# yeyupiaoling/MASR

Measured on NVIDIA H100. Metric: audio_seconds_per_second, higher is better.
Workload: dtype f32 (GEMMs: fp16x2-split operands on wgmma, fp32 accumulate; fp32-grade results)

## Files before the change

### masr_b200/csrc/ffn_tc.cu

```cuda
#include <cuda.h>
#include <cuda_fp16.h>
#include <stdlib.h>
#include <string.h>

#include "tc_common.cuh"

namespace masr {

namespace {

constexpr int FM = 64;
constexpr int FD = 256;
constexpr int FHC = 128;
constexpr int FBK = 32;
constexpr int F_STAGES = 3;
constexpr int F_STAGE_BYTES = 32768;
constexpr int F_H_BYTES = FM * FHC * 2 * 2;
constexpr int F_SUM_BYTES = FM * FD * 4;
constexpr int F_THREADS = 384;
constexpr int F_PRODUCER_REGS = 40, F_CONSUMER_REGS = 232;
constexpr uint32_t F_TX_A = 2 * FM * FBK * 2 + 2 * FHC * FBK * 2;
constexpr uint32_t F_TX_B = 2 * FD * FBK * 2;
constexpr size_t kFfnSmem = F_STAGES * F_STAGE_BYTES + 2 * F_H_BYTES + F_SUM_BYTES + 1024 + 256;
static_assert(kFfnSmem <= 232448, "ffn_tc shared memory exceeds the 227 KB per-CTA limit of sm_90");
static_assert(F_PRODUCER_REGS * 128 + F_CONSUMER_REGS * 256 <= 65536, "register file of the SM");

struct FfnMaps {
    CUtensorMap xh, xl;
    CUtensorMap w1h, w1l;
    CUtensorMap w2h, w2l;
};

struct FfnParams {
    const void* w[4];
    const float* b1;
    const float* b2;
    float* x;
    int64_t ldx;
    int M, F;
    float alpha;
    int flags;
};

constexpr int FFN_NO_LOADS = 1, FFN_NO_MMA = 2, FFN_NO_EPILOGUE = 4;

__device__ __forceinline__ void wgmma_m64n64k16_ss(float (&d)[32], uint64_t da, uint64_t db, uint32_t scale_d) {
    asm volatile(
        "{\n\t"
        ".reg .pred p;\n\t"
        "setp.ne.b32 p, %34, 0;\n\t"
        "wgmma.mma_async.sync.aligned.m64n64k16.f32.f16.f16 "
        "{%0, %1, %2, %3, %4, %5, %6, %7, %8, %9, %10, %11, %12, %13, %14, %15, "
        "%16, %17, %18, %19, %20, %21, %22, %23, %24, %25, %26, %27, %28, %29, %30, %31}, %32, %33, p, 1, 1, 0, 0;\n\t"
        "}"
        : "+f"(d[0]), "+f"(d[1]), "+f"(d[2]), "+f"(d[3]), "+f"(d[4]), "+f"(d[5]), "+f"(d[6]), "+f"(d[7]), "+f"(d[8]),
          "+f"(d[9]), "+f"(d[10]), "+f"(d[11]), "+f"(d[12]), "+f"(d[13]), "+f"(d[14]), "+f"(d[15]), "+f"(d[16]),
          "+f"(d[17]), "+f"(d[18]), "+f"(d[19]), "+f"(d[20]), "+f"(d[21]), "+f"(d[22]), "+f"(d[23]), "+f"(d[24]),
          "+f"(d[25]), "+f"(d[26]), "+f"(d[27]), "+f"(d[28]), "+f"(d[29]), "+f"(d[30]), "+f"(d[31])
        : "l"(da), "l"(db), "r"(scale_d));
}

__device__ __forceinline__ void bar_consumers() { asm volatile("bar.sync 1, 256;" ::: "memory"); }

template <bool PROBE>
__global__ void __launch_bounds__(F_THREADS, 1) ffn_tc_kernel(const __grid_constant__ FfnMaps maps, FfnParams p) {
    const bool no_loads = PROBE && (p.flags & FFN_NO_LOADS), no_mma = PROBE && (p.flags & FFN_NO_MMA);
    const bool no_epilogue = PROBE && (p.flags & FFN_NO_EPILOGUE);
    extern __shared__ uint8_t smem_raw[];
    uint8_t* smem = reinterpret_cast<uint8_t*>((reinterpret_cast<uintptr_t>(smem_raw) + 1023) & ~uintptr_t(1023));
    uint8_t* hbuf = smem + F_STAGES * F_STAGE_BYTES;
    uint8_t* sum = hbuf + 2 * F_H_BYTES;
    uint64_t* full_bar = reinterpret_cast<uint64_t*>(sum + F_SUM_BYTES);
    uint64_t* empty_bar = full_bar + F_STAGES;

    const int warp = threadIdx.x >> 5, lane = threadIdx.x & 31;
    const int nrb = (p.M + FM - 1) / FM;
    const int nch = p.F / FHC;

    if (warp == 8 && lane == 0) {
        tma_prefetch_desc(&maps.xh); tma_prefetch_desc(&maps.xl); tma_prefetch_desc(&maps.w1h);
        tma_prefetch_desc(&maps.w1l); tma_prefetch_desc(&maps.w2h); tma_prefetch_desc(&maps.w2l);
        for (int s = 0; s < F_STAGES; ++s) { mbar_init(&full_bar[s], 1); mbar_init(&empty_bar[s], 8); }
        asm volatile("fence.mbarrier_init.release.cluster;" ::: "memory");
        const uint32_t wbytes = (uint32_t)p.F * FD * 2;
        const uint32_t share = ((wbytes + gridDim.x - 1) / gridDim.x + 15) & ~15u;
        const uint32_t off = share * blockIdx.x;
        if (!no_loads && off < wbytes)
            for (int t = 0; t < 4; ++t)
                asm volatile("cp.async.bulk.prefetch.L2.global [%0], %1;"
                             ::"l"(static_cast<const uint8_t*>(p.w[t]) + off), "r"(min(share, wbytes - off)) : "memory");
    }
    __syncthreads();
    pdl_wait();
    pdl_launch_dependents();

    if (warp >= 8) {
        setmaxnreg_dec<F_PRODUCER_REGS>();
        if (warp == 8 && elect_one_sync()) {
            uint32_t kg = 0;
            auto acquire = [&](uint32_t tx) {
                const uint32_t s = kg % F_STAGES;
                mbar_wait(&empty_bar[s], ((kg / F_STAGES) & 1) ^ 1);
                if (no_loads) mbar_arrive(&full_bar[s]);
                else mbar_expect_tx(&full_bar[s], tx);
                ++kg;
                return s;
            };
            auto load_a = [&](int m0, int j) {
                const int n0 = j * FHC;
#pragma unroll 1
                for (int kb = 0; kb < FD / FBK; ++kb) {
                    const uint32_t s = acquire(F_TX_A);
                    if (no_loads) continue;
                    uint8_t* st = smem + s * F_STAGE_BYTES;
                    tma_load_2d(&maps.xh, &full_bar[s], st, kb * FBK, m0);
                    tma_load_2d(&maps.xl, &full_bar[s], st + 4096, kb * FBK, m0);
                    tma_load_2d(&maps.w1h, &full_bar[s], st + 8192, kb * FBK, n0);
                    tma_load_2d(&maps.w1l, &full_bar[s], st + 16384, kb * FBK, n0);
                }
            };
            for (int rb = blockIdx.x; rb < nrb; rb += gridDim.x) {
                load_a(rb * FM, 0);
                for (int j = 0; j < nch; ++j) {
                    if (j + 1 < nch) load_a(rb * FM, j + 1);
#pragma unroll 1
                    for (int kb = 0; kb < FHC / FBK; ++kb) {
                        const uint32_t s = acquire(F_TX_B);
                        if (no_loads) continue;
                        uint8_t* st = smem + s * F_STAGE_BYTES;
                        tma_load_2d(&maps.w2h, &full_bar[s], st, j * FHC + kb * FBK, 0);
                        tma_load_2d(&maps.w2l, &full_bar[s], st + F_STAGE_BYTES / 2, j * FHC + kb * FBK, 0);
                    }
                }
            }
        }
        __syncwarp();
    } else {
        setmaxnreg_inc<F_CONSUMER_REGS>();
        const int wg = warp >> 2, wi = warp & 3, q = lane & 3;
        const int tid = threadIdx.x & 127;
        const uint32_t h_base = smem_u32(hbuf);
        const uint32_t sum_base = smem_u32(sum) + wg * (F_SUM_BYTES / 2) + tid * 8;
        const uint32_t is_lane0 = lane == 0;
        auto release = [&](uint32_t s) {
            asm volatile("{\n\t.reg .pred p;\n\tsetp.ne.u32 p, %1, 0;\n\t@p mbarrier.arrive.shared::cta.b64 _, [%0];\n\t}"
                         ::"r"(smem_u32(&empty_bar[s])), "r"(is_lane0) : "memory");
        };
        float acc1[32], cor1[32], acc2[64], cor2[64];
        uint32_t kg = 0;
        int pend = -1;
        auto next_stage = [&]() {
            const uint32_t s = kg % F_STAGES;
            mbar_wait(&full_bar[s], (kg / F_STAGES) & 1);
            ++kg;
            return s;
        };
        auto retire = [&](uint32_t s) {
            wgmma_wait<1>();
            reg_fence(acc1); reg_fence(cor1); reg_fence(acc2); reg_fence(cor2);
            if (pend >= 0) release((uint32_t)pend);
            pend = (int)s;
        };
        auto phase_a = [&](int kb_begin, int kb_end) {
#pragma unroll 1
            for (int kb = kb_begin; kb < kb_end; ++kb) {
                const uint32_t s = next_stage();
                const uint32_t sa = smem_u32(smem + s * F_STAGE_BYTES);
                const uint64_t dXh = gmma_desc_sw64(sa), dXl = gmma_desc_sw64(sa + 4096);
                const uint64_t dWh = gmma_desc_sw64(sa + 8192 + wg * 4096), dWl = gmma_desc_sw64(sa + 16384 + wg * 4096);
                reg_fence(acc1); reg_fence(cor1);
                wgmma_fence();
#pragma unroll
                for (int ks = 0; ks < FBK / 16; ++ks) {
                    if (no_mma) break;
                    const uint64_t adv = (uint64_t)(ks * 2);
                    const uint32_t first = (kb | ks) ? 1u : 0u;
                    wgmma_m64n64k16_ss(acc1, dXh + adv, dWh + adv, first);
                    wgmma_m64n64k16_ss(cor1, dXh + adv, dWl + adv, first);
                    wgmma_m64n64k16_ss(cor1, dXl + adv, dWh + adv, 1u);
                }
                wgmma_commit();
                retire(s);
            }
        };
        auto phase_b = [&](int j, uint32_t hb, int kb) {
            const uint32_t s = next_stage();
            const uint32_t sa = smem_u32(smem + s * F_STAGE_BYTES);
            const uint64_t dWh = gmma_desc_sw64(sa + wg * 8192), dWl = gmma_desc_sw64(sa + F_STAGE_BYTES / 2 + wg * 8192);
            const uint64_t dHh = gmma_desc_sw64(hb + kb * 8192), dHl = gmma_desc_sw64(hb + kb * 8192 + 4096);
            reg_fence(acc2); reg_fence(cor2);
            wgmma_fence();
#pragma unroll
            for (int ks = 0; ks < FBK / 16; ++ks) {
                if (no_mma) break;
                const uint64_t adv = (uint64_t)(ks * 2);
                wgmma_m64n128k16_ss(acc2, dHh + adv, dWh + adv, ((j & 1) | kb | ks) ? 1u : 0u);
                wgmma_m64n128k16_ss(cor2, dHh + adv, dWl + adv, (j | kb | ks) ? 1u : 0u);
                wgmma_m64n128k16_ss(cor2, dHl + adv, dWh + adv, 1u);
            }
            wgmma_commit();
            retire(s);
        };
        const int r_lo = 16 * wi + (lane >> 2);
        auto load_b1 = [&](int j, int sl, float2 (&bb)[2]) {
            const float* b = p.b1 + j * FHC + 64 * wg + 16 * sl + 2 * q;
            bb[0] = __ldg(reinterpret_cast<const float2*>(b));
            bb[1] = __ldg(reinterpret_cast<const float2*>(b + 8));
        };
        auto store_hidden = [&](uint32_t hb, int sl, const float2 (&bb)[2]) {
            if (no_epilogue) return;
#pragma unroll
            for (int i = 2 * sl; i < 2 * sl + 2; ++i)
#pragma unroll
                for (int hh = 0; hh < 2; ++hh) {
                    float v0 = fmaf(cor1[4 * i + 2 * hh], kLoInv, acc1[4 * i + 2 * hh]);
                    float v1 = fmaf(cor1[4 * i + 2 * hh + 1], kLoInv, acc1[4 * i + 2 * hh + 1]);
                    v0 += bb[i - 2 * sl].x; v1 += bb[i - 2 * sl].y;
                    float e0, e1;
                    mul2(e0, e1, v0, v1, -1.4426950408889634f, -1.4426950408889634f);
                    e0 = ex2_approx(e0); e1 = ex2_approx(e1);
                    add2(e0, e1, e0, e1, 1.0f, 1.0f);
                    e0 = rcp_approx(e0); e1 = rcp_approx(e1);
                    mul2(v0, v1, v0, v1, e0, e1);
                    __half2 h2, l2;
                    split_f16x2(v0, v1, h2, l2);
                    const int r = r_lo + 8 * hh, c = 64 * wg + 8 * i + 2 * q;
                    const uint32_t a = hb + (c >> 5) * 8192 + r * 64 + ((((c & 31) >> 3) ^ ((r >> 1) & 3)) << 4) + (c & 7) * 2;
                    asm volatile("st.shared.b32 [%0], %1;" ::"r"(a), "r"(*reinterpret_cast<uint32_t*>(&h2)) : "memory");
                    asm volatile("st.shared.b32 [%0], %1;" ::"r"(a + 4096), "r"(*reinterpret_cast<uint32_t*>(&l2)) : "memory");
                }
        };
        auto fence_h = [&]() { asm volatile("fence.proxy.async.shared::cta;" ::: "memory"); };
        auto drain = [&]() {
            wgmma_wait<0>();
            reg_fence(acc1); reg_fence(cor1); reg_fence(acc2); reg_fence(cor2);
            if (pend >= 0) release((uint32_t)pend);
            pend = -1;
        };

        auto add_sum = [&](int j) {
#pragma unroll
            for (int i = 0; i < 16; ++i)
#pragma unroll
                for (int hh = 0; hh < 2; ++hh) {
                    float x0 = acc2[4 * i + 2 * hh], x1 = acc2[4 * i + 2 * hh + 1];
                    const uint32_t a = sum_base + (i * 2 + hh) * 1024;
                    if (j > 1) {
                        float s0, s1;
                        asm volatile("ld.shared.v2.f32 {%0, %1}, [%2];" : "=f"(s0), "=f"(s1) : "r"(a) : "memory");
                        x0 = s0 + x0; x1 = s1 + x1;
                    }
                    asm volatile("st.shared.v2.f32 [%0], {%1, %2};" ::"r"(a), "f"(x0), "f"(x1) : "memory");
                }
        };
        auto write_out = [&](int m0) {
            const float* b2 = p.b2 + 128 * wg + 2 * q;
#pragma unroll
            for (int i = 0; i < 16; ++i) {
                const float2 bv = __ldg(reinterpret_cast<const float2*>(b2 + 8 * i));
#pragma unroll
                for (int hh = 0; hh < 2; ++hh) {
                    float x0 = acc2[4 * i + 2 * hh], x1 = acc2[4 * i + 2 * hh + 1];
                    if (nch > 2) {
                        float s0, s1;
                        asm volatile("ld.shared.v2.f32 {%0, %1}, [%2];" : "=f"(s0), "=f"(s1) : "r"(sum_base + (i * 2 + hh) * 1024) : "memory");
                        x0 = s0 + x0; x1 = s1 + x1;
                    }
                    x0 = fmaf(cor2[4 * i + 2 * hh], kLoInv, x0);
                    x1 = fmaf(cor2[4 * i + 2 * hh + 1], kLoInv, x1);
                    x0 += bv.x; x1 += bv.y;
                    const int row = m0 + r_lo + 8 * hh;
                    if (row < p.M) {
                        float2* xp = reinterpret_cast<float2*>(p.x + (int64_t)row * p.ldx + 128 * wg + 8 * i + 2 * q);
                        const float2 r = *xp;
                        x0 = r.x + p.alpha * x0;
                        x1 = r.y + p.alpha * x1;
                        *xp = make_float2(x0, x1);
                    }
                }
            }
        };

#pragma unroll 1
        for (int rb = blockIdx.x; rb < nrb; rb += gridDim.x) {
            phase_a(0, FD / FBK);
            drain();
#pragma unroll
            for (int sl = 0; sl < 4; ++sl) {
                float2 bb[2];
                load_b1(0, sl, bb);
                store_hidden(h_base, sl, bb);
            }
            fence_h();
            phase_a(0, FD / FBK);
            drain();
            bar_consumers();
#pragma unroll 1
            for (int j = 0; j < nch; ++j) {
                const bool next = j + 1 < nch, a2 = j + 2 < nch;
                const uint32_t hb = h_base + (j & 1) * F_H_BYTES, hn = h_base + ((j + 1) & 1) * F_H_BYTES;
#pragma unroll
                for (int kb = 0; kb < FHC / FBK; ++kb) {
                    float2 bb[2];
                    if (next) load_b1(j + 1, kb, bb);
                    phase_b(j, hb, kb);
                    if (next) store_hidden(hn, kb, bb);
                }
                if (next) fence_h();
                if (a2) phase_a(0, 1);
                else drain();
                if ((j & 1) && j + 1 < nch) add_sum(j);
                if (j == nch - 1) write_out(rb * FM);
                if (a2) phase_a(1, FD / FBK);
                if (next) bar_consumers();
                drain();
            }
        }
    }
    __syncthreads();
}

int ffn_map(CUtensorMap* map, const void* ptr, int64_t rows, int64_t K, int64_t ld, int box_rows) {
    EncodeTiledFn fn = get_encode_fn();
    if (!fn) { set_last_error("cuTensorMapEncodeTiled entry point unavailable"); return MASR_ERR_INTERNAL; }
    cuuint64_t dims[2] = {(cuuint64_t)K, (cuuint64_t)rows};
    cuuint64_t strides[1] = {(cuuint64_t)ld * 2};
    cuuint32_t box[2] = {(cuuint32_t)FBK, (cuuint32_t)box_rows};
    cuuint32_t estr[2] = {1, 1};
    CUresult r = fn(map, CU_TENSOR_MAP_DATA_TYPE_FLOAT16, 2, const_cast<void*>(ptr), dims, strides, box, estr,
                    CU_TENSOR_MAP_INTERLEAVE_NONE, CU_TENSOR_MAP_SWIZZLE_64B, CU_TENSOR_MAP_L2_PROMOTION_L2_128B,
                    CU_TENSOR_MAP_FLOAT_OOB_FILL_NONE);
    if (r != CUDA_SUCCESS) { set_last_error("cuTensorMapEncodeTiled failed (%d) rows=%lld K=%lld ld=%lld", (int)r, (long long)rows, (long long)K, (long long)ld); return MASR_ERR_INTERNAL; }
    return MASR_OK;
}

bool g_ffn_attr_set[64] = {false};

}

}

using namespace masr;

extern "C" int masr_ffn_tc_f16x2(const void* Ah, const void* Al, int64_t lda, const void* W1h, const void* W1l, const float* b1,
                                 const void* W2h, const void* W2l, const float* b2, float* x, int64_t ldx, int M, int D, int F,
                                 float alpha, void* stream) {
    if (M == 0) return MASR_OK;
    MASR_REQUIRE(Ah && Al && W1h && W1l && b1 && W2h && W2l && b2 && x, "masr_ffn_tc_f16x2: null pointer");
    MASR_REQUIRE(M > 0, "masr_ffn_tc_f16x2: M=%d", M);
    MASR_REQUIRE(D == FD, "masr_ffn_tc_f16x2: D=%d unsupported (this build: %d)", D, FD);
    MASR_REQUIRE(F > 0 && F % 256 == 0, "masr_ffn_tc_f16x2: F=%d must be a positive multiple of 256", F);
    MASR_REQUIRE(lda >= D && lda % 8 == 0, "masr_ffn_tc_f16x2: lda=%lld must be >= %d and a multiple of 8", (long long)lda, D);
    MASR_REQUIRE(ldx >= D && ldx % 2 == 0, "masr_ffn_tc_f16x2: ldx=%lld must be >= %d and even", (long long)ldx, D);
    MASR_REQUIRE(((reinterpret_cast<uintptr_t>(Ah) | reinterpret_cast<uintptr_t>(Al) | reinterpret_cast<uintptr_t>(W1h) |
                   reinterpret_cast<uintptr_t>(W1l) | reinterpret_cast<uintptr_t>(W2h) | reinterpret_cast<uintptr_t>(W2l)) & 15) == 0 &&
                 ((reinterpret_cast<uintptr_t>(x) | reinterpret_cast<uintptr_t>(b1) | reinterpret_cast<uintptr_t>(b2)) & 7) == 0,
                 "masr_ffn_tc_f16x2: misaligned pointer");
    FfnMaps maps;
    memset(&maps, 0, sizeof(maps));
    int rc;
    if ((rc = ffn_map(&maps.xh, Ah, M, D, lda, FM))) return rc;
    if ((rc = ffn_map(&maps.xl, Al, M, D, lda, FM))) return rc;
    if ((rc = ffn_map(&maps.w1h, W1h, F, D, D, FHC))) return rc;
    if ((rc = ffn_map(&maps.w1l, W1l, F, D, D, FHC))) return rc;
    if ((rc = ffn_map(&maps.w2h, W2h, D, F, F, FD))) return rc;
    if ((rc = ffn_map(&maps.w2l, W2l, D, F, F, FD))) return rc;
    int dev = 0;
    cudaGetDevice(&dev);
    if (dev < 0 || dev >= 64) dev = 0;
    void (*const kernels[2])(FfnMaps, FfnParams) = {ffn_tc_kernel<false>, ffn_tc_kernel<true>};
    if (!g_ffn_attr_set[dev]) {
        for (auto k : kernels) {
            cudaError_t e = cudaFuncSetAttribute(k, cudaFuncAttributeMaxDynamicSharedMemorySize, (int)kFfnSmem);
            if (e != cudaSuccess) { set_last_error("ffn_tc smem attr: %s", cudaGetErrorString(e)); return (int)e; }
        }
        g_ffn_attr_set[dev] = true;
    }
    int sms = 0;
    if (cudaDeviceGetAttribute(&sms, cudaDevAttrMultiProcessorCount, dev) != cudaSuccess || sms <= 0) sms = 132;
    const int nrb = (M + FM - 1) / FM;
    const char* env = getenv("MASR_FFN_FLAGS");
    const int flags = env ? atoi(env) : 0;
    FfnParams p{{W1h, W1l, W2h, W2l}, b1, b2, x, ldx, M, F, alpha, flags};
    const dim3 grid(nrb < sms ? nrb : sms);
    launch_pdl(kernels[flags ? 1 : 0], grid, dim3(F_THREADS), kFfnSmem, (cudaStream_t)stream, maps, p);
    return check_launch("ffn_tc_kernel");
}
```

### masr_b200/csrc/tc_common.cuh

```cuda
#pragma once
#include <cuda.h>
#include <cuda_fp16.h>
#include <mutex>

#include "common.cuh"

namespace masr {

constexpr float kLoScale = 2048.0f, kLoInv = 1.0f / 2048.0f;

__device__ __forceinline__ uint32_t smem_u32(const void* p) { return (uint32_t)__cvta_generic_to_shared(p); }

__device__ __forceinline__ void mbar_init(uint64_t* bar, uint32_t count) {
    asm volatile("mbarrier.init.shared::cta.b64 [%0], %1;" ::"r"(smem_u32(bar)), "r"(count));
}
__device__ __forceinline__ void mbar_expect_tx(uint64_t* bar, uint32_t bytes) {
    asm volatile("mbarrier.arrive.expect_tx.shared::cta.b64 _, [%0], %1;" ::"r"(smem_u32(bar)), "r"(bytes) : "memory");
}
__device__ __forceinline__ void mbar_wait(uint64_t* bar, uint32_t parity) {
    asm volatile(
        "{\n\t"
        ".reg .pred P1;\n\t"
        "WAIT_LOOP:\n\t"
        "mbarrier.try_wait.parity.shared::cta.b64 P1, [%0], %1;\n\t"
        "@P1 bra DONE;\n\t"
        "bra WAIT_LOOP;\n\t"
        "DONE:\n\t"
        "}" ::"r"(smem_u32(bar)), "r"(parity) : "memory");
}
__device__ __forceinline__ void tma_load_2d(const CUtensorMap* map, uint64_t* bar, void* smem_dst, int c0, int c1) {
    asm volatile(
        "cp.async.bulk.tensor.2d.shared::cluster.global.mbarrier::complete_tx::bytes [%0], [%1, {%3, %4}], [%2];"
        ::"r"(smem_u32(smem_dst)), "l"(map), "r"(smem_u32(bar)), "r"(c0), "r"(c1) : "memory");
}
__device__ __forceinline__ void tma_prefetch_desc(const CUtensorMap* map) {
    asm volatile("prefetch.tensormap [%0];" ::"l"(map) : "memory");
}
__device__ __forceinline__ bool elect_one_sync() {
    uint32_t pred = 0, laneid = 0;
    asm volatile(
        "{\n\t"
        ".reg .b32 %%rx;\n\t"
        ".reg .pred %%px;\n\t"
        "elect.sync %%rx|%%px, %2;\n\t"
        "@%%px mov.s32 %1, 1;\n\t"
        "mov.s32 %0, %%rx;\n\t"
        "}"
        : "+r"(laneid), "+r"(pred)
        : "r"(0xFFFFFFFFu));
    return pred != 0;
}

__device__ __forceinline__ void wgmma_fence() { asm volatile("wgmma.fence.sync.aligned;" ::: "memory"); }
__device__ __forceinline__ void wgmma_commit() { asm volatile("wgmma.commit_group.sync.aligned;" ::: "memory"); }
template <int N>
__device__ __forceinline__ void wgmma_wait() { asm volatile("wgmma.wait_group.sync.aligned %0;" ::"n"(N) : "memory"); }
template <int R>
__device__ __forceinline__ void reg_fence(float (&d)[R]) {
#pragma unroll
    for (int i = 0; i < R; ++i) asm volatile("" : "+f"(d[i])::"memory");
}
__device__ __forceinline__ void wgmma_m64n128k16_ss(float (&d)[64], uint64_t da, uint64_t db, uint32_t scale_d) {
    asm volatile(
        "{\n\t"
        ".reg .pred p;\n\t"
        "setp.ne.b32 p, %66, 0;\n\t"
        "wgmma.mma_async.sync.aligned.m64n128k16.f32.f16.f16 "
        "{%0, %1, %2, %3, %4, %5, %6, %7, %8, %9, %10, %11, %12, %13, %14, %15, "
        "%16, %17, %18, %19, %20, %21, %22, %23, %24, %25, %26, %27, %28, %29, %30, %31, "
        "%32, %33, %34, %35, %36, %37, %38, %39, %40, %41, %42, %43, %44, %45, %46, %47, "
        "%48, %49, %50, %51, %52, %53, %54, %55, %56, %57, %58, %59, %60, %61, %62, %63}, %64, %65, p, 1, 1, 0, 0;\n\t"
        "}"
        : "+f"(d[0]), "+f"(d[1]), "+f"(d[2]), "+f"(d[3]), "+f"(d[4]), "+f"(d[5]), "+f"(d[6]), "+f"(d[7]), "+f"(d[8]),
          "+f"(d[9]), "+f"(d[10]), "+f"(d[11]), "+f"(d[12]), "+f"(d[13]), "+f"(d[14]), "+f"(d[15]), "+f"(d[16]),
          "+f"(d[17]), "+f"(d[18]), "+f"(d[19]), "+f"(d[20]), "+f"(d[21]), "+f"(d[22]), "+f"(d[23]), "+f"(d[24]),
          "+f"(d[25]), "+f"(d[26]), "+f"(d[27]), "+f"(d[28]), "+f"(d[29]), "+f"(d[30]), "+f"(d[31]), "+f"(d[32]),
          "+f"(d[33]), "+f"(d[34]), "+f"(d[35]), "+f"(d[36]), "+f"(d[37]), "+f"(d[38]), "+f"(d[39]), "+f"(d[40]),
          "+f"(d[41]), "+f"(d[42]), "+f"(d[43]), "+f"(d[44]), "+f"(d[45]), "+f"(d[46]), "+f"(d[47]), "+f"(d[48]),
          "+f"(d[49]), "+f"(d[50]), "+f"(d[51]), "+f"(d[52]), "+f"(d[53]), "+f"(d[54]), "+f"(d[55]), "+f"(d[56]),
          "+f"(d[57]), "+f"(d[58]), "+f"(d[59]), "+f"(d[60]), "+f"(d[61]), "+f"(d[62]), "+f"(d[63])
        : "l"(da), "l"(db), "r"(scale_d));
}
template <int R>
__device__ __forceinline__ void setmaxnreg_inc() { asm volatile("setmaxnreg.inc.sync.aligned.u32 %0;" ::"n"(R)); }
template <int R>
__device__ __forceinline__ void setmaxnreg_dec() { asm volatile("setmaxnreg.dec.sync.aligned.u32 %0;" ::"n"(R)); }

__device__ __forceinline__ uint64_t gmma_desc_sw64(uint32_t smem_addr) {
    uint64_t d = 0;
    d |= (uint64_t)((smem_addr & 0x3FFFF) >> 4);
    d |= (uint64_t)1 << 16;
    d |= (uint64_t)(512 >> 4) << 32;
    d |= (uint64_t)2 << 62;
    return d;
}

__device__ __forceinline__ void add2(float& d0, float& d1, float a0, float a1, float b0, float b1) { d0 = a0 + b0; d1 = a1 + b1; }
__device__ __forceinline__ void sub2(float& d0, float& d1, float a0, float a1, float b0, float b1) { d0 = a0 - b0; d1 = a1 - b1; }
__device__ __forceinline__ void mul2(float& d0, float& d1, float a0, float a1, float b0, float b1) { d0 = a0 * b0; d1 = a1 * b1; }
__device__ __forceinline__ void split_f16(float x, __half& h, __half& l) {
    h = __float2half_rn(x);
    l = __float2half_rn((x - __half2float(h)) * kLoScale);
}
__device__ __forceinline__ void split_f16x2(float x0, float x1, __half2& h, __half2& l) {
    h = __floats2half2_rn(x0, x1);
    const float2 hf = __half22float2(h);
    float d0, d1;
    sub2(d0, d1, x0, x1, hf.x, hf.y);
    mul2(d0, d1, d0, d1, kLoScale, kLoScale);
    l = __floats2half2_rn(d0, d1);
}

__device__ __forceinline__ void mbar_arrive(uint64_t* bar) {
    asm volatile("mbarrier.arrive.shared::cta.b64 _, [%0];" ::"r"(smem_u32(bar)) : "memory");
}

__device__ __forceinline__ void sts128(uint32_t a, const uint4& v) {
    asm volatile("st.shared.v4.b32 [%0], {%1, %2, %3, %4};" ::"r"(a), "r"(v.x), "r"(v.y), "r"(v.z), "r"(v.w) : "memory");
}
__device__ __forceinline__ uint4 lds128(uint32_t a) {
    uint4 v;
    asm volatile("ld.shared.v4.b32 {%0, %1, %2, %3}, [%4];" : "=r"(v.x), "=r"(v.y), "=r"(v.z), "=r"(v.w) : "r"(a) : "memory");
    return v;
}

typedef CUresult (*EncodeTiledFn)(CUtensorMap*, CUtensorMapDataType, cuuint32_t, void*, const cuuint64_t*, const cuuint64_t*,
                                  const cuuint32_t*, const cuuint32_t*, CUtensorMapInterleave, CUtensorMapSwizzle,
                                  CUtensorMapL2promotion, CUtensorMapFloatOOBfill);

inline EncodeTiledFn get_encode_fn() {
    static EncodeTiledFn fn = nullptr;
    static std::once_flag once;
    std::call_once(once, [] {
        void* p = nullptr;
        cudaDriverEntryPointQueryResult qres;
        if (cudaGetDriverEntryPoint("cuTensorMapEncodeTiled", &p, cudaEnableDefault, &qres) == cudaSuccess &&
            qres == cudaDriverEntryPointSuccess)
            fn = reinterpret_cast<EncodeTiledFn>(p);
    });
    return fn;
}

}
```

Before: 52670.

## Multicast FFN weight tiles across a 2-CTA cluster via TMA

Launches the fused FFN kernel as 2-CTA clusters. Each CTA loads half of every W1/W2 weight tile and multicasts it to both CTAs, which halves per-CTA weight traffic from L2. Empty barriers become cluster-wide, so each consumer warp arrives on both CTAs' barriers. The trade-off is lockstep coupling between paired CTAs, extra remote-barrier traffic, and a grid sized from cluster occupancy. An odd row-block count gives a duplicate clamped load in the producer, while the consumer uses the unclamped row index.

```diff
diff --git a/masr_b200/csrc/ffn_tc.cu b/masr_b200/csrc/ffn_tc.cu
--- a/masr_b200/csrc/ffn_tc.cu
+++ b/masr_b200/csrc/ffn_tc.cu
@@ -18,6 +18,7 @@
 constexpr int F_H_BYTES = FM * FHC * 2 * 2;
 constexpr int F_SUM_BYTES = FM * FD * 4;
 constexpr int F_THREADS = 384;
+constexpr int F_CLUSTER = 2;
 constexpr int F_PRODUCER_REGS = 40, F_CONSUMER_REGS = 232;
 constexpr uint32_t F_TX_A = 2 * FM * FBK * 2 + 2 * FHC * FBK * 2;
 constexpr uint32_t F_TX_B = 2 * FD * FBK * 2;
@@ -76,11 +77,14 @@
     const int warp = threadIdx.x >> 5, lane = threadIdx.x & 31;
     const int nrb = (p.M + FM - 1) / FM;
     const int nch = p.F / FHC;
+    const uint32_t rank = blockIdx.x % F_CLUSTER;
+    const int cluster = blockIdx.x / F_CLUSTER, clusters = gridDim.x / F_CLUSTER;
+    const int npairs = (nrb + F_CLUSTER - 1) / F_CLUSTER;
 
     if (warp == 8 && lane == 0) {
         tma_prefetch_desc(&maps.xh); tma_prefetch_desc(&maps.xl); tma_prefetch_desc(&maps.w1h);
         tma_prefetch_desc(&maps.w1l); tma_prefetch_desc(&maps.w2h); tma_prefetch_desc(&maps.w2l);
-        for (int s = 0; s < F_STAGES; ++s) { mbar_init(&full_bar[s], 1); mbar_init(&empty_bar[s], 8); }
+        for (int s = 0; s < F_STAGES; ++s) { mbar_init(&full_bar[s], 1); mbar_init(&empty_bar[s], 8 * F_CLUSTER); }
         asm volatile("fence.mbarrier_init.release.cluster;" ::: "memory");
         const uint32_t wbytes = (uint32_t)p.F * FD * 2;
         const uint32_t share = ((wbytes + gridDim.x - 1) / gridDim.x + 15) & ~15u;
@@ -90,7 +94,7 @@
                 asm volatile("cp.async.bulk.prefetch.L2.global [%0], %1;"
                              ::"l"(static_cast<const uint8_t*>(p.w[t]) + off), "r"(min(share, wbytes - off)) : "memory");
     }
-    __syncthreads();
+    cluster_sync();
     pdl_wait();
     pdl_launch_dependents();
 
@@ -106,8 +110,9 @@
                 ++kg;
                 return s;
             };
+            constexpr uint16_t both = (1u << F_CLUSTER) - 1;
             auto load_a = [&](int m0, int j) {
-                const int n0 = j * FHC;
+                const int n0 = j * FHC + (FHC / F_CLUSTER) * rank;
 #pragma unroll 1
                 for (int kb = 0; kb < FD / FBK; ++kb) {
                     const uint32_t s = acquire(F_TX_A);
@@ -115,21 +120,23 @@
                     uint8_t* st = smem + s * F_STAGE_BYTES;
                     tma_load_2d(&maps.xh, &full_bar[s], st, kb * FBK, m0);
                     tma_load_2d(&maps.xl, &full_bar[s], st + 4096, kb * FBK, m0);
-                    tma_load_2d(&maps.w1h, &full_bar[s], st + 8192, kb * FBK, n0);
-                    tma_load_2d(&maps.w1l, &full_bar[s], st + 16384, kb * FBK, n0);
+                    tma_load_2d_multicast(&maps.w1h, &full_bar[s], st + 8192 + 4096 * rank, kb * FBK, n0, both);
+                    tma_load_2d_multicast(&maps.w1l, &full_bar[s], st + 16384 + 4096 * rank, kb * FBK, n0, both);
                 }
             };
-            for (int rb = blockIdx.x; rb < nrb; rb += gridDim.x) {
-                load_a(rb * FM, 0);
+            for (int pair = cluster; pair < npairs; pair += clusters) {
+                const int m0 = min(pair * F_CLUSTER + (int)rank, nrb - 1) * FM;
+                load_a(m0, 0);
                 for (int j = 0; j < nch; ++j) {
-                    if (j + 1 < nch) load_a(rb * FM, j + 1);
+                    if (j + 1 < nch) load_a(m0, j + 1);
 #pragma unroll 1
                     for (int kb = 0; kb < FHC / FBK; ++kb) {
                         const uint32_t s = acquire(F_TX_B);
                         if (no_loads) continue;
                         uint8_t* st = smem + s * F_STAGE_BYTES;
-                        tma_load_2d(&maps.w2h, &full_bar[s], st, j * FHC + kb * FBK, 0);
-                        tma_load_2d(&maps.w2l, &full_bar[s], st + F_STAGE_BYTES / 2, j * FHC + kb * FBK, 0);
+                        const int k0 = j * FHC + kb * FBK, r0 = (FD / F_CLUSTER) * rank;
+                        tma_load_2d_multicast(&maps.w2h, &full_bar[s], st + 8192 * rank, k0, r0, both);
+                        tma_load_2d_multicast(&maps.w2l, &full_bar[s], st + F_STAGE_BYTES / 2 + 8192 * rank, k0, r0, both);
                     }
                 }
             }
@@ -142,9 +149,10 @@
         const uint32_t h_base = smem_u32(hbuf);
         const uint32_t sum_base = smem_u32(sum) + wg * (F_SUM_BYTES / 2) + tid * 8;
         const uint32_t is_lane0 = lane == 0;
+        const uint32_t empty0 = cluster_map(smem_u32(empty_bar), 0), empty1 = cluster_map(smem_u32(empty_bar), 1);
         auto release = [&](uint32_t s) {
-            asm volatile("{\n\t.reg .pred p;\n\tsetp.ne.u32 p, %1, 0;\n\t@p mbarrier.arrive.shared::cta.b64 _, [%0];\n\t}"
-                         ::"r"(smem_u32(&empty_bar[s])), "r"(is_lane0) : "memory");
+            mbar_arrive_cluster(empty0 + 8 * s, is_lane0);
+            mbar_arrive_cluster(empty1 + 8 * s, is_lane0);
         };
         float acc1[32], cor1[32], acc2[64], cor2[64];
         uint32_t kg = 0;
@@ -282,7 +290,8 @@
         };
 
 #pragma unroll 1
-        for (int rb = blockIdx.x; rb < nrb; rb += gridDim.x) {
+        for (int pair = cluster; pair < npairs; pair += clusters) {
+            const int rb = pair * F_CLUSTER + (int)rank;
             phase_a(0, FD / FBK);
             drain();
 #pragma unroll
@@ -317,7 +326,7 @@
             }
         }
     }
-    __syncthreads();
+    cluster_sync();
 }
 
 int ffn_map(CUtensorMap* map, const void* ptr, int64_t rows, int64_t K, int64_t ld, int box_rows) {
@@ -335,6 +344,7 @@
 }
 
 bool g_ffn_attr_set[64] = {false};
+int g_ffn_clusters[64][2] = {};
 
 }
 
@@ -361,10 +371,10 @@
     int rc;
     if ((rc = ffn_map(&maps.xh, Ah, M, D, lda, FM))) return rc;
     if ((rc = ffn_map(&maps.xl, Al, M, D, lda, FM))) return rc;
-    if ((rc = ffn_map(&maps.w1h, W1h, F, D, D, FHC))) return rc;
-    if ((rc = ffn_map(&maps.w1l, W1l, F, D, D, FHC))) return rc;
-    if ((rc = ffn_map(&maps.w2h, W2h, D, F, F, FD))) return rc;
-    if ((rc = ffn_map(&maps.w2l, W2l, D, F, F, FD))) return rc;
+    if ((rc = ffn_map(&maps.w1h, W1h, F, D, D, FHC / F_CLUSTER))) return rc;
+    if ((rc = ffn_map(&maps.w1l, W1l, F, D, D, FHC / F_CLUSTER))) return rc;
+    if ((rc = ffn_map(&maps.w2h, W2h, D, F, F, FD / F_CLUSTER))) return rc;
+    if ((rc = ffn_map(&maps.w2l, W2l, D, F, F, FD / F_CLUSTER))) return rc;
     int dev = 0;
     cudaGetDevice(&dev);
     if (dev < 0 || dev >= 64) dev = 0;
@@ -376,13 +386,36 @@
         }
         g_ffn_attr_set[dev] = true;
     }
-    int sms = 0;
-    if (cudaDeviceGetAttribute(&sms, cudaDevAttrMultiProcessorCount, dev) != cudaSuccess || sms <= 0) sms = 132;
-    const int nrb = (M + FM - 1) / FM;
     const char* env = getenv("MASR_FFN_FLAGS");
     const int flags = env ? atoi(env) : 0;
+    const int kind = flags ? 1 : 0;
+    cudaLaunchConfig_t cfg = {};
+    cfg.blockDim = dim3(F_THREADS);
+    cfg.dynamicSmemBytes = kFfnSmem;
+    cudaLaunchAttribute attr[2];
+    attr[0].id = cudaLaunchAttributeClusterDimension;
+    attr[0].val.clusterDim.x = F_CLUSTER;
+    attr[0].val.clusterDim.y = 1;
+    attr[0].val.clusterDim.z = 1;
+    attr[1].id = cudaLaunchAttributeProgrammaticStreamSerialization;
+    attr[1].val.programmaticStreamSerializationAllowed = 1;
+    cfg.attrs = attr;
+    cfg.numAttrs = 1;
+    if (!g_ffn_clusters[dev][kind]) {
+        cfg.gridDim = dim3(F_CLUSTER);
+        int n = 0;
+        const cudaError_t e = cudaOccupancyMaxActiveClusters(&n, kernels[kind], &cfg);
+        if (e != cudaSuccess || n <= 0) {
+            set_last_error("ffn_tc: no cluster of %d CTAs fits (%s)", F_CLUSTER, cudaGetErrorString(e));
+            return e != cudaSuccess ? (int)e : MASR_ERR_INTERNAL;
+        }
+        g_ffn_clusters[dev][kind] = n;
+    }
+    const int npairs = ((M + FM - 1) / FM + F_CLUSTER - 1) / F_CLUSTER;
     FfnParams p{{W1h, W1l, W2h, W2l}, b1, b2, x, ldx, M, F, alpha, flags};
-    const dim3 grid(nrb < sms ? nrb : sms);
-    launch_pdl(kernels[flags ? 1 : 0], grid, dim3(F_THREADS), kFfnSmem, (cudaStream_t)stream, maps, p);
+    cfg.gridDim = dim3(F_CLUSTER * (npairs < g_ffn_clusters[dev][kind] ? npairs : g_ffn_clusters[dev][kind]));
+    cfg.stream = (cudaStream_t)stream;
+    cfg.numAttrs = pdl_enabled() ? 2 : 1;
+    cudaLaunchKernelEx(&cfg, kernels[kind], maps, p);
     return check_launch("ffn_tc_kernel");
 }
diff --git a/masr_b200/csrc/tc_common.cuh b/masr_b200/csrc/tc_common.cuh
--- a/masr_b200/csrc/tc_common.cuh
+++ b/masr_b200/csrc/tc_common.cuh
@@ -32,6 +32,21 @@
     asm volatile(
         "cp.async.bulk.tensor.2d.shared::cluster.global.mbarrier::complete_tx::bytes [%0], [%1, {%3, %4}], [%2];"
         ::"r"(smem_u32(smem_dst)), "l"(map), "r"(smem_u32(bar)), "r"(c0), "r"(c1) : "memory");
+}
+__device__ __forceinline__ void tma_load_2d_multicast(const CUtensorMap* map, uint64_t* bar, void* smem_dst, int c0, int c1,
+                                                      uint16_t cta_mask) {
+    asm volatile(
+        "cp.async.bulk.tensor.2d.shared::cluster.global.mbarrier::complete_tx::bytes.multicast::cluster"
+        " [%0], [%1, {%3, %4}], [%2], %5;"
+        ::"r"(smem_u32(smem_dst)), "l"(map), "r"(smem_u32(bar)), "r"(c0), "r"(c1), "h"(cta_mask) : "memory");
+}
+__device__ __forceinline__ uint32_t cluster_map(uint32_t a, uint32_t rank) {
+    uint32_t r;
+    asm volatile("mapa.shared::cluster.u32 %0, %1, %2;" : "=r"(r) : "r"(a), "r"(rank));
+    return r;
+}
+__device__ __forceinline__ void cluster_sync() {
+    asm volatile("barrier.cluster.arrive.release.aligned;\n\tbarrier.cluster.wait.acquire.aligned;" ::: "memory");
 }
 __device__ __forceinline__ void tma_prefetch_desc(const CUtensorMap* map) {
     asm volatile("prefetch.tensormap [%0];" ::"l"(map) : "memory");
@@ -114,6 +129,10 @@
 __device__ __forceinline__ void mbar_arrive(uint64_t* bar) {
     asm volatile("mbarrier.arrive.shared::cta.b64 _, [%0];" ::"r"(smem_u32(bar)) : "memory");
 }
+__device__ __forceinline__ void mbar_arrive_cluster(uint32_t a, uint32_t pred) {
+    asm volatile("{\n\t.reg .pred p;\n\tsetp.ne.u32 p, %1, 0;\n\t@p mbarrier.arrive.shared::cluster.b64 _, [%0];\n\t}"
+                 ::"r"(a), "r"(pred) : "memory");
+}
 
 __device__ __forceinline__ void sts128(uint32_t a, const uint4& v) {
     asm volatile("st.shared.v4.b32 [%0], {%1, %2, %3, %4};" ::"r"(a), "r"(v.x), "r"(v.y), "r"(v.z), "r"(v.w) : "memory");
```

Result: faster. 54470 (median of 6 runs) (+3.4%).
